# wei-zeng98/piano-a2s

Measured on AMD Instinct MI355X. Metric: training clips/sec (12 s, 5-bar), higher is better.
Workload: dtype f32

## Files before the change

piano_a2s_amd/csrc/a2s_api.hip:

```cpp
#define A2S_SWITCHES_IMPL
#include "a2s_internal.h"

thread_local char a2s_err_msg[512] = {0};
long long a2s_launch_counter = 0;

#define ST ((hipStream_t)stream)

extern "C" {

const char* a2s_last_error(void) { return a2s_err_msg; }
int a2s_version(void) { return 1; }
long long a2s_launch_count(void) { return __atomic_load_n(&a2s_launch_counter, __ATOMIC_RELAXED); }

int a2s_gemm_f32(void* stream, int M, int N, int K, float alpha, const float* A, long sAm, long sAk, const float* B, long sBk,
                 long sBn, float beta, float* C, long ldc, const float* bias, int act, int batch, long bsA, long bsB, long bsC,
                 int splitk, float* workspace, size_t workspace_bytes) {
    return a2s_gemm_impl(ST, M, N, K, alpha, A, sAm, sAk, B, sBk, sBn, beta, C, ldc, bias, act, batch, bsA, bsB, bsC, splitk,
                         workspace, workspace_bytes);
}
int a2s_gemm_f32_affine(void* stream, int M, int N, int K, float alpha, const float* A, long sAm, long sAk, const float* B, long sBk,
                        long sBn, float beta, float* C, long ldc, const float* bias, int act, int batch, long bsA, long bsB, long bsC,
                        int splitk, float* workspace, size_t workspace_bytes, const float* a_scale, const float* a_shift, int a_period,
                        const float* b_scale, const float* b_shift, int b_period) {
    return a2s_gemm_affine_impl(ST, M, N, K, alpha, A, sAm, sAk, B, sBk, sBn, beta, C, ldc, bias, act, batch, bsA, bsB, bsC, splitk,
                                workspace, workspace_bytes, a_scale, a_shift, a_period, b_scale, b_shift, b_period,
                                nullptr, nullptr, nullptr, nullptr, nullptr, nullptr, 0, 0, nullptr, nullptr);
}
int a2s_gemm_f32_affine_scaled(void* stream, int M, int N, int K, float alpha, const float* A, long sAm, long sAk, const float* B, long sBk,
                               long sBn, float beta, float* C, long ldc, const float* bias, int act, int batch, long bsA, long bsB, long bsC,
                               int splitk, float* workspace, size_t workspace_bytes, const float* a_scale, const float* a_shift, int a_period,
                               const float* b_scale, const float* b_shift, int b_period, const float* a_absmax, const float* b_absmax) {
    return a2s_gemm_affine_impl(ST, M, N, K, alpha, A, sAm, sAk, B, sBk, sBn, beta, C, ldc, bias, act, batch, bsA, bsB, bsC, splitk,
                                workspace, workspace_bytes, a_scale, a_shift, a_period, b_scale, b_shift, b_period,
                                nullptr, nullptr, nullptr, nullptr, nullptr, nullptr, 0, 1, a_absmax, b_absmax);
}
int a2s_gemm_f32_bnstats_scaled(void* stream, int M, int N, int K, const float* A, long sAm, long sAk, const float* B, long sBk, long sBn, float* C, long ldc,
                                const float* y, const float* mean, const float* invstd, const float* scale, const float* shift, int period, float* partial,
                                const float* a_absmax, const float* b_absmax) {
    return a2s_gemm_affine_impl(ST, M, N, K, 1.f, A, sAm, sAk, B, sBk, sBn, 0.f, C, ldc, nullptr, 0, 1, 0, 0, 0, 1, nullptr, 0,
                                nullptr, nullptr, 0, nullptr, nullptr, 0, y, mean, invstd, scale, shift, partial, period, 1, a_absmax, b_absmax);
}
int a2s_absmax(void* stream, const float* x, long n, float* out) { return a2s_absmax_impl(ST, x, n, out); }
int a2s_linear_dgrad_bnstats(void* stream, int M, int N, int K, const float* dz, long lda, const float* Wt, float* da, long ldc, const float* y,
                             const float* mean, const float* invstd, const float* scale, const float* shift, int period, float* partial,
                             const float* dz_absmax, const float* w_absmax, float* workspace, size_t workspace_bytes, float* da_absmax_out) {
    return a2s_linear_dgrad_bnstats_impl(ST, M, N, K, dz, lda, Wt, 1, K, da, ldc, y, mean, invstd, scale, shift, period, partial, dz_absmax, w_absmax,
                                         workspace, workspace_bytes, da_absmax_out);
}
size_t a2s_linear_dgrad_ws_bytes(int N, int K) { return a2s_linear_dgrad_ws_bytes_impl(N, K); }
int a2s_linear_fwd(void* stream, int M, int N, int K, const float* y, long lda, const float* W, float* z, long ldc, const float* scale, const float* shift,
                   int period, const float* y_absmax, const float* w_absmax, float* workspace, size_t workspace_bytes) {
    return a2s_linear_fwd_impl(ST, M, N, K, y, lda, W, z, ldc, scale, shift, period, y_absmax, w_absmax, workspace, workspace_bytes);
}
int a2s_linear_wgrad(void* stream, int M, int N, int K, const float* dz, long ldz, const float* y, long lda, float* G, long ldg, const float* scale,
                     const float* shift, int period, const float* dz_absmax, const float* y_absmax, float* workspace, size_t workspace_bytes) {
    return a2s_linear_wgrad_impl(ST, M, N, K, dz, ldz, y, lda, G, ldg, scale, shift, period, dz_absmax, y_absmax, workspace, workspace_bytes);
}
size_t a2s_linear_wgrad_ws_bytes(int M, int K) { return a2s_linear_wgrad_ws_bytes_impl(M, K); }
int a2s_linear_wgrad_eligible(int M, int N, int K, int period) { return a2s_linear_wgrad_ok(M, N, K, 256, 4, 4, period, nullptr, nullptr, nullptr) ? 1 : 0; }
int a2s_tallk_wgrad(void* stream, int M, int Np, int K, const float* P, long ldp, const float* A, long lda, float* G, long ldg, int transposed, float* bias,
                    const float* p_absmax, const float* a_absmax, float* workspace, size_t workspace_bytes) {
    return a2s_tallk_wgrad_impl(ST, M, Np, K, P, ldp, A, lda, G, ldg, transposed, bias, p_absmax, a_absmax, workspace, workspace_bytes);
}
size_t a2s_tallk_wgrad_ws_bytes(int M, int Np, int K) { return a2s_tallk_wgrad_ws_bytes_impl(M, Np, K); }
int a2s_tallk_wgrad_eligible(int M, int Np, int K, long ldp, long lda, long ldg, int transposed) {
    return a2s_tallk_wgrad_ok(M, Np, K, ldp, lda, ldg, transposed, nullptr, nullptr, nullptr, nullptr) ? 1 : 0;
}
int a2s_linear_fwd_eligible(int M, int N, int K, int period) { return a2s_linear_fwd_ok(M, N, K, 4, 4, period, nullptr, nullptr, nullptr) ? 1 : 0; }
int a2s_linear_dgrad_blocks(int M) { return a2s_linear_dgrad_blocks_impl(M); }
int a2s_linear_dgrad_eligible(int M, int N, int K, int period) {
    return a2s_linear_dgrad_ok(M, N, K, 4, 1, K, 4, period, nullptr, nullptr, nullptr, nullptr) ? 1 : 0;
}
int a2s_gemm_f32_bnstats(void* stream, int M, int N, int K, const float* A, long sAm, long sAk, const float* B, long sBk, long sBn, float* C, long ldc,
                         const float* y, const float* mean, const float* invstd, const float* scale, const float* shift, int period, float* partial) {
    return a2s_gemm_affine_impl(ST, M, N, K, 1.f, A, sAm, sAk, B, sBk, sBn, 0.f, C, ldc, nullptr, 0, 1, 0, 0, 0, 1, nullptr, 0,
                                nullptr, nullptr, 0, nullptr, nullptr, 0, y, mean, invstd, scale, shift, partial, period, 0, nullptr, nullptr);
}
int a2s_gemm_bnstats_blocks(int M, int period) { return a2s_cdiv(M, 128) * a2s_gemm_bnstats_slots(period); }
size_t a2s_gemm_workspace_bytes(int M, int N, int batch, int splitk) { return a2s_gemm_workspace_bytes_impl(M, N, batch, splitk); }
int a2s_gemm_pick_splitk(int M, int N, int K, int batch) { return a2s_gemm_pick_splitk_impl(M, N, K, batch); }
void a2s_gemm_debug_tile(int cfg) { a2s_gemm_debug_tile_impl(cfg); }
size_t a2s_note_step_workspace_floats(int H, int E) { return a2s_note_step_workspace_floats_impl(H, E); }
int a2s_debug_set(const char* key, int value) {
    if (!key) return A2S_ERR_ARG;
    const int id = a2s_switch_find(key);
    if (id >= 0) { a2s_switch_store(id, value); return A2S_OK; }
    if (!strcmp(key, "attn_deferred_fast")) { a2s_attn_deferred_fast = value ? 1 : 0; return A2S_OK; }
    if (!strcmp(key, "tallk_wgrad")) { a2s_tallk_wgrad_on = value ? 1 : 0; return A2S_OK; }
    if (!strcmp(key, "tallk_wgrad_max_splits")) { a2s_tallk_wgrad_max_splits = value > 0 ? value : 0; return A2S_OK; }
    if (!strcmp(key, "gemm_tile")) { a2s_gemm_debug_tile_impl(value); return A2S_OK; }
    snprintf(a2s_err_msg, sizeof(a2s_err_msg), "a2s_debug_set: unknown key %s", key);
    return A2S_ERR_ARG;
}
int a2s_env_check(void) {
    if (const char* e = a2s_switch_env_error()) A2S_FAIL(A2S_ERR_ARG, "%s: expected a decimal number >= 0", e);
    return A2S_OK;
}

int a2s_persist_abort_latch(void* device_word) { a2s_persist_latch_set(device_word); return A2S_OK; }

int a2s_debug_get(const char* key) {
    if (!key) return -1;
    const int id = a2s_switch_find(key);
    if (id == A2S_SW_attn_pair_fused_rows) return a2s_attn_pair_fused_rows();
    if (id >= 0) return a2s_sw((a2s_switch)id);
    if (!strcmp(key, "attn_pair_launches")) return (int)a2s_attn_pair_launches();
    if (!strcmp(key, "attn_pair_bwd_launches")) return (int)a2s_attn_pair_bwd_launches();
    if (!strcmp(key, "attn_deferred_fast")) return a2s_attn_deferred_fast;
    if (!strcmp(key, "tallk_wgrad")) return a2s_tallk_wgrad_on;
    if (!strcmp(key, "tallk_wgrad_max_splits")) return a2s_tallk_wgrad_max_splits;
    if (!strcmp(key, "tallk_wgrad_launches")) return (int)a2s_tallk_wgrad_launches();
    if (!strcmp(key, "attn_dk_ahead_launches")) return (int)a2s_attn_dk_ahead_launches();
    if (!strcmp(key, "attn_denc_launches")) return (int)a2s_attn_denc_launches();
    if (!strcmp(key, "dec_mid_launches")) return a2s_dec_mid_launches();
    if (!strcmp(key, "dec_persist_launches")) return a2s_dec_persist_launches();
    if (!strcmp(key, "edit_distance_launches")) return (int)a2s_edit_distance_launches();
    if (!strcmp(key, "conv_rows16_c20_launches")) return (int)a2s_conv_rows16_c20_launches();
    if (!strcmp(key, "device_cus")) return a2s_device_geometry().cus;
    if (!strcmp(key, "device_xccs")) return a2s_device_geometry().xccs;
    return -1;
}

int a2s_conv3x3(void* stream, const float* x, const float* w, float* y, const float* in_scale, const float* in_shift,
                float* stat_partial, int B, int T, int F, int Cin, int Cout, int flip, float* workspace) {
    return a2s_conv3x3_impl(ST, x, w, y, in_scale, in_shift, stat_partial, B, T, F, Cin, Cout, flip, workspace, nullptr, nullptr, nullptr, nullptr, nullptr, nullptr,
                            nullptr, nullptr);
}
int a2s_conv3x3_ranged(void* stream, const float* x, const float* w, float* y, const float* in_scale, const float* in_shift, const float* in_absmax,
                       float* stat_partial, float* out_absmax, int B, int T, int F, int Cin, int Cout, float* workspace) {
    return a2s_conv3x3_impl(ST, x, w, y, in_scale, in_shift, stat_partial, B, T, F, Cin, Cout, 0, workspace, nullptr, nullptr, nullptr, nullptr, nullptr, nullptr,
                            in_absmax, out_absmax);
}
int a2s_conv3x3_dgrad_bnstats(void* stream, const float* dy, const float* w, float* g, const float* yl, const float* yl_mean, const float* yl_invstd,
                              const float* yl_scale, const float* yl_shift, float* stat_partial, int B, int T, int F, int Cin, int Cout,
                              float* workspace) {
    if (!yl) { snprintf(a2s_err_msg, sizeof(a2s_err_msg), "conv3x3_dgrad_bnstats: yl is required"); return A2S_ERR_ARG; }
    return a2s_conv3x3_impl(ST, dy, w, g, nullptr, nullptr, stat_partial, B, T, F, Cin, Cout, 1, workspace, yl, yl_mean, yl_invstd, yl_scale, yl_shift, nullptr, nullptr, nullptr);
}
int a2s_conv3x3_dgrad_bnstats_scaled(void* stream, const float* dy, const float* w, float* g, const float* yl, const float* yl_mean, const float* yl_invstd,
                                     const float* yl_scale, const float* yl_shift, float* stat_partial, int B, int T, int F, int Cin, int Cout,
                                     float* workspace, const float* dy_absmax) {
    if (!yl) { snprintf(a2s_err_msg, sizeof(a2s_err_msg), "conv3x3_dgrad_bnstats_scaled: yl is required"); return A2S_ERR_ARG; }
    return a2s_conv3x3_impl(ST, dy, w, g, nullptr, nullptr, stat_partial, B, T, F, Cin, Cout, 1, workspace, yl, yl_mean, yl_invstd, yl_scale, yl_shift, dy_absmax, nullptr, nullptr);
}
int a2s_conv3x3_dgrad_bnstats_ranged(void* stream, const float* dy, const float* w, float* g, const float* yl, const float* yl_mean, const float* yl_invstd,
                                     const float* yl_scale, const float* yl_shift, float* stat_partial, int B, int T, int F, int Cin, int Cout,
                                     float* workspace, const float* dy_absmax, float* g_absmax_out) {
    if (!yl) { snprintf(a2s_err_msg, sizeof(a2s_err_msg), "conv3x3_dgrad_bnstats_ranged: yl is required"); return A2S_ERR_ARG; }
    return a2s_conv3x3_impl(ST, dy, w, g, nullptr, nullptr, stat_partial, B, T, F, Cin, Cout, 1, workspace, yl, yl_mean, yl_invstd, yl_scale, yl_shift, dy_absmax, nullptr, g_absmax_out);
}
int a2s_bn_bwd_from_partial(void* stream, const float* g, const float* x, const float* mean, const float* invstd, const float* scale, const float* shift,
                            float* dgamma, float* dbeta, float* dx, const float* partial, int nblocks, float* c12, long rows, int C, int F) {
    return a2s_bn_bwd_from_partial_impl(ST, g, x, mean, invstd, scale, shift, dgamma, dbeta, dx, partial, nblocks, c12, rows, C, F, nullptr);
}
int a2s_bn_bwd_from_partial_amax(void* stream, const float* g, const float* x, const float* mean, const float* invstd, const float* scale, const float* shift,
                                 float* dgamma, float* dbeta, float* dx, const float* partial, int nblocks, float* c12, long rows, int C, int F,
                                 float* dx_absmax) {
    return a2s_bn_bwd_from_partial_impl(ST, g, x, mean, invstd, scale, shift, dgamma, dbeta, dx, partial, nblocks, c12, rows, C, F, dx_absmax);
}
size_t a2s_conv3x3_workspace_floats(int Cin) { return a2s_conv3x3_workspace_floats_impl(Cin); }
int a2s_conv3x3_stat_blocks(int B, int T, int F, int Cin) { return a2s_conv3x3_stat_blocks_impl(B, T, F, Cin); }
int a2s_bn_finalize(void* stream, const float* partial, int nblocks, int C, double count, const float* gamma, const float* beta,
                    float* running_mean, float* running_var, long long* nbt, float* mean, float* invstd, float* scale,
                    float* shift, float eps, float momentum, int training) {
    return a2s_bn_finalize_impl(ST, partial, nblocks, C, count, gamma, beta, running_mean, running_var, nbt, mean, invstd, scale,
                                shift, eps, momentum, training);
}
int a2s_bn_relu_apply(void* stream, const float* x, float* y, const float* scale, const float* shift, long n, int C, int F) {
    return a2s_bn_relu_apply_impl(ST, x, y, scale, shift, n, C, F);
}
int a2s_col_stats(void* stream, const float* x, float* partial, long rows, int C, int rows_per_block) {
    return a2s_col_stats_impl(ST, x, partial, rows, C, rows_per_block);
}
int a2s_bn1d_relu_dropout(void* stream, const float* x, float* y, const float* scale, const float* shift, const uint8_t* keep_mask,
                          float inv_keep, long n, int C) {
    return a2s_bn1d_relu_dropout_impl(ST, x, y, scale, shift, keep_mask, inv_keep, n, C);
}
int a2s_gru_gates_fwd(void* stream, const float* gi, long ldgi, const float* gh, long ldgh, const float* hprev, long ldhp,
                      float* hout, long ldho, float* hout2, long ldho2, float* save, int R, int H) {
    return a2s_gru_gates_fwd_impl(ST, gi, ldgi, gh, ldgh, hprev, ldhp, hout, ldho, hout2, ldho2, save, R, H);
}
int a2s_gru_seq_fwd(void* stream, const float* gi_all, long gi_bstride, long gi_tstride, const float* w_hh, const float* b_hh,
                    float* out, long out_bstride, long out_tstride, float* hbuf, float* gh, float* save, float* hn, int B, int T,
                    int H, int reverse, float* workspace, size_t workspace_bytes) {
    return a2s_gru_seq_fwd_impl(ST, gi_all, gi_bstride, gi_tstride, w_hh, b_hh, out, out_bstride, out_tstride, hbuf, gh, save, hn,
                                B, T, H, reverse, workspace, workspace_bytes);
}
int a2s_attn_step_fwd(void* stream, const float* keys, const float* enc, const float* q, long ldq, const float* v, float* ctx,
                      long ldctx, float* ctx2, long ldctx2, float* attw, int B, int T, int H, const int* n_done, int n_rows_total, float* workspace) {
    return a2s_attn_step_fwd_impl(ST, keys, enc, q, ldq, v, ctx, ldctx, ctx2, ldctx2, attw, B, T, H, n_done, n_rows_total, workspace, nullptr);
}
int a2s_attn_step_fwd_rows(void* stream, const float* keys, const float* enc, const float* q, long ldq, const float* v, float* ctx,
                           long ldctx, float* ctx2, long ldctx2, float* attw, int R, int T, int H, float* workspace, int n_clips,
                           const int* clip_order, const int* clip_rank, const int* row_until, int n_active, int step) {
// ... 258 lines not shown
```

piano_a2s_amd/csrc/a2s_internal.h:

```cpp
#pragma once
#include "a2s_common.h"
#include "../../include/a2s.h"
#include "a2s_switches.h"

static inline int a2s_attn_pair_fused_rows(void) {
    const int cap = a2s_sw(A2S_SW_dec_fused_max_rows), v = a2s_sw(A2S_SW_attn_pair_fused_rows);
    return v < cap ? v : cap;
}
static inline unsigned a2s_persist_dbg(void) {
    return (a2s_sw(A2S_SW_persist_force_agent) ? PERSIST_DBG_FORCE_AGENT : 0u) | (a2s_sw(A2S_SW_persist_inject_abort) ? PERSIST_DBG_INJECT_ABORT : 0u);
}

int a2s_absmax_impl(hipStream_t st, const float* x, long n, float* out);
size_t a2s_gemm_workspace_bytes_impl(int M, int N, int batch, int splitk);
int a2s_gemm_pick_splitk_impl(int M, int N, int K, int batch);
int a2s_gemm_bnstats_slots(int period);
void a2s_gemm_debug_tile_impl(int cfg);
int a2s_gemm_affine_impl(hipStream_t st, int M, int N, int K, float alpha, const float* A, long sAm, long sAk,
    const float* B, long sBk, long sBn, float beta, float* C, long ldc, const float* bias, int act,
    int batch, long bsA, long bsB, long bsC, int splitk, float* ws, size_t ws_bytes,
    const float* a_scale, const float* a_shift, int a_period, const float* b_scale, const float* b_shift, int b_period,
    const float* ep_y, const float* ep_mean, const float* ep_invstd, const float* ep_scale, const float* ep_shift,
    float* ep_partial, int ep_period, int two_term, const float* a_absmax, const float* b_absmax);
int a2s_gemm_impl(hipStream_t st, int M, int N, int K, float alpha, const float* A, long sAm, long sAk,
    const float* B, long sBk, long sBn, float beta, float* C, long ldc, const float* bias, int act,
    int batch, long bsA, long bsB, long bsC, int splitk, float* ws, size_t ws_bytes);

size_t a2s_linear_dgrad_ws_bytes_impl(int N, int K);
int a2s_linear_dgrad_blocks_impl(int M);
bool a2s_linear_dgrad_ok(int M, int N, int K, long lda, long sBk, long sBn, long ldc, int period, const void* A, const void* B, const void* C, const void* y);
int a2s_linear_dgrad_bnstats_impl(hipStream_t st, int M, int N, int K, const float* A, long lda, const float* Wt, long sBk, long sBn, float* C, long ldc,
    const float* ep_y, const float* mean, const float* invstd, const float* scale, const float* shift, int period,
    float* partial, const float* a_absmax, const float* b_absmax, float* ws, size_t ws_bytes, float* c_absmax_out);
bool a2s_linear_fwd_ok(int M, int N, int K, long lda, long ldc, int period, const void* A, const void* W, const void* C);
int a2s_linear_fwd_impl(hipStream_t st, int M, int N, int K, const float* A, long lda, const float* W, float* C, long ldc, const float* a_scale,
    const float* a_shift, int period, const float* a_absmax, const float* w_absmax, float* ws, size_t ws_bytes);
size_t a2s_linear_wgrad_ws_bytes_impl(int M, int K);
bool a2s_linear_wgrad_ok(int M, int N, int K, long ldz, long lda, long ldg, int period, const void* dz, const void* A, const void* G);
int a2s_linear_wgrad_impl(hipStream_t st, int M, int N, int K, const float* dz, long ldz, const float* A, long lda, float* G, long ldg, const float* a_scale,
    const float* a_shift, int period, const float* dz_absmax, const float* a_absmax, float* ws, size_t ws_bytes);
extern int a2s_tallk_wgrad_on;
extern int a2s_tallk_wgrad_max_splits;
long a2s_tallk_wgrad_launches(void);
size_t a2s_tallk_wgrad_ws_bytes_impl(int M, int Np, int K);
bool a2s_tallk_wgrad_ok(int M, int Np, int K, long ldp, long lda, long ldg, int transposed, const void* P, const void* A, const void* G, const void* bias);
int a2s_tallk_wgrad_impl(hipStream_t st, int M, int Np, int K, const float* P, long ldp, const float* A, long lda, float* G, long ldg, int transposed,
    float* bias, const float* p_absmax, const float* a_absmax, float* ws, size_t ws_bytes);

int a2s_act_bound_impl(hipStream_t st, const float* scale, const float* shift, const float* absmax, int C, float* out);
size_t a2s_conv3x3_workspace_floats_impl(int Cin);
int a2s_conv3x3_impl(hipStream_t st, const float* x, const float* w, float* y, const float* in_scale,
    const float* in_shift, float* stat_partial, int B, int T, int F, int Cin, int Cout, int flip, float* ws,
    const float* yl, const float* yl_mean, const float* yl_invstd, const float* yl_scale, const float* yl_shift,
    const float* x_absmax, const float* in_absmax, float* out_absmax);
int a2s_conv3x3_stat_blocks_impl(int B, int T, int F, int Cin);
int a2s_bn_finalize_impl(hipStream_t st, const float* partial, int nblocks, int C, double count, const float* gamma,
    const float* beta, float* running_mean, float* running_var, long long* nbt, float* mean,
    float* invstd, float* scale, float* shift, float eps, float momentum, int training);
int a2s_bn_relu_apply_impl(hipStream_t st, const float* x, float* y, const float* scale, const float* shift, long n, int C, int F);
int a2s_col_stats_impl(hipStream_t st, const float* x, float* partial, long rows, int C, int rows_per_block);
int a2s_bn1d_relu_dropout_impl(hipStream_t st, const float* x, float* y, const float* scale, const float* shift,
    const uint8_t* mask, float inv_keep, long n, int C);
size_t a2s_conv3x3_wgrad_workspace_bytes_impl(int Cin, int Cout);
int a2s_conv3x3_wgrad_impl(hipStream_t st, const float* dy, const float* x, const float* in_scale, const float* in_shift, float* dW,
    float* ws, size_t ws_bytes, int B, int T, int F, int Cin, int Cout, const float* bn_y, const float* bn_mean,
    const float* bn_invstd, const float* bn_scale, const float* bn_shift, const float* bn_c12, float* dy_out,
    const float* dy_absmax, const float* act_absmax);
int a2s_bn_bwd_impl(hipStream_t st, const float* g, const float* x, const float* mean, const float* invstd, const float* scale,
    const float* shift, const uint8_t* mask, float inv_keep, float* dgamma, float* dbeta, float* dx, float* partial,
    float* c12, long rows, int C, int F, float* dx_absmax);
int a2s_bn_bwd_from_partial_impl(hipStream_t st, const float* g, const float* x, const float* mean, const float* invstd, const float* scale,
    const float* shift, float* dgamma, float* dbeta, float* dx, const float* partial, int nblocks, float* c12,
    long rows, int C, int F, float* dx_absmax);
int a2s_bn_bwd_stats_impl(hipStream_t st, const float* g, const float* x, const float* mean, const float* invstd, const float* scale,
    const float* shift, const uint8_t* mask, float inv_keep, float* partial, float* sums, long rows, int C, int F);
int a2s_bn_bwd_apply_impl(hipStream_t st, const float* g, const float* x, const float* mean, const float* invstd, const float* scale,
    const float* shift, const uint8_t* mask, float inv_keep, const float* sums_local, const float* sums_global,
    double count_global, float* dgamma, float* dbeta, float* dx, float* c12, long rows, int C, int F);
int a2s_bn_bwd_sums_from_partial_impl(hipStream_t st, const float* partial, int nblocks, int C, float* sums);
int a2s_bn_bwd_c12_from_sums_impl(hipStream_t st, const float* sums_local, const float* sums_global, double count_global, float* dgamma, float* dbeta,
    float* c12, int C);
size_t a2s_bn_bwd_partial_floats_impl(long rows, int C, int F);

int a2s_channel_absmax_impl(hipStream_t st, const float* x, long rows, int C, int F, float* out);
bool a2s_conv_rows_eligible(int F, int Cin);
int a2s_conv_rows_blocks(int B, int T, int F);
size_t a2s_conv_rows_workspace_floats(int Cin);
long a2s_conv_rows16_c20_launches(void);
int a2s_conv3x3_rows_impl(hipStream_t st, const float* x, const float* w, float* y, const float* in_scale, const float* in_shift,
    const float* in_absmax, float* stat_partial, float* out_absmax, int B, int T, int F, int Cin, int Cout, int flip,
    float* ws, const float* yl, const float* yl_mean, const float* yl_invstd, const float* yl_scale, const float* yl_shift,
    const float* x_absmax);

bool a2s_wgrad_rows_eligible(int F, int Cin, int Cout);
int a2s_conv3x3_wgrad_rows_bn_impl(hipStream_t st, const float* g, const float* y, const float* mean, const float* invstd, const float* scale,
    const float* shift, const float* c12, const float* g_absmax, int g_absmax_n, const float* y_absmax, float* dz_out,
    float* dz_absmax_out, const float* x, const float* in_scale, const float* in_shift, float* dW, float* ws, size_t ws_bytes,
    int B, int T, int F, int Cin, int Cout, const float* act_absmax);
int a2s_conv3x3_wgrad_rows_impl(hipStream_t st, const float* dy, const float* x, const float* in_scale, const float* in_shift, float* dW, float* ws,
    size_t ws_bytes, int B, int T, int F, int Cin, int Cout, const float* dy_absmax, const float* act_absmax);

struct StepFinArgs {
    const float* logits; long ldl;
    float* probs; long probs_bstride;
    const long long* gt; long gt_bstride;
    const float* emb;
    float* xnext; long ldx;
    const uint8_t* drop; float inv_keep;
    int* argmax_out; long am_bstride;
    int* eos_seen; long long* lengths; int* n_done; int* steps_exec;
    const int* t_base;
    const int* row_until;
    int n_clips;
    int R, V, E, t, teacher_force, eos_id, max_t;
};
struct a2s_grammar_ref { const signed char* next; int n_states; int* row_state; };
int a2s_gru_gates_fwd_impl(hipStream_t st, const float* gi, long ldgi, const float* gh, long ldgh, const float* hprev,
    long ldhp, float* hout, long ldho, float* hout2, long ldho2, float* save, int R, int H);
int a2s_gru_bptt_step_impl(hipStream_t st, const float* dgh, const float* w_hh_t, const float* dhz_in, const float* dout, long ld_dout,
    const float* save, const float* hprev, long ld_hprev, float* dgi, long ld_dgi, float* dgh_out, float* dgh2,
    long ld_dgh2, float* dhz_out, int R, int H);
int a2s_skinny_gemm_acc_impl(hipStream_t st, const float* A, long lda, const float* Bt, long ldb, float* Cm, long ldc, int R, int N, int K);
int a2s_gru_seq_fwd_impl(hipStream_t st, const float* gi_all, long gi_bstride, long gi_tstride, const float* w_hh,
    const float* b_hh, float* out, long out_bstride, long out_tstride, float* hbuf, float* gh,
    float* save, float* hn, int B, int T, int H, int reverse, float* ws, size_t ws_bytes);
int a2s_attn_step_fwd_impl(hipStream_t st, const float* Kmat, const float* enc, const float* q, long ldq, const float* v,
// ... 161 lines not shown
```

piano_a2s_amd/csrc/a2s_linear.hip:

```cpp
#include "a2s_internal.h"

#define LIN_BM 128
#define LIN_K 256
#define LIN_RS 288
#define LIN_NTH 512
#define LIN_LDS (2 * 2 * LIN_BM * LIN_RS)

typedef unsigned lu32x4 __attribute__((ext_vector_type(4)));

struct LinDgradArgs {
    const float* A; long lda;
    const unsigned char* planes;
    float* C; long ldc;
    const float* ep_y;
    const float* mean; const float* invstd; const float* scale; const float* shift;
    float* partial;
    const float* a_absmax; const float* b_absmax;
    int M, N, period, channels;
    float* c_absmax_out;
};

__global__ __launch_bounds__(256) void lin_pack_planes_k(const float* __restrict__ W, long ld, int N, int K, const float* __restrict__ absmax,
                                                         unsigned char* __restrict__ out) {
    const long id = (long)blockIdx.x * 256 + threadIdx.x;
// ... 264 lines not shown
#pragma unroll
        for (int sp = 0; sp < 2; ++sp)
#pragma unroll
            for (int q = 0; q < 2; ++q) af[sp][q] = *reinterpret_cast<const lu32x4*>(st + (sp * LIN_BM + (qt * 2 + q) * 16 + lr) * LF_RS + h * 64 + lk * 16);
    };
    auto multiply = [&](int qt, const lu32x4 (&af)[2][2], const lu32x4 (&b)[4][2]) {
#define LR_PRODUCT(SA, SB)                                                                                                        \
        _Pragma("unroll") for (int nt = 0; nt < 4; ++nt)                                                                          \
            _Pragma("unroll") for (int q = 0; q < 2; ++q)                                                                         \
                acc[qt * 2 + q][nt] = __builtin_amdgcn_mfma_f32_16x16x32_f16(__builtin_bit_cast(f16x8, b[nt][SB]),                \
                                                                             __builtin_bit_cast(f16x8, af[SA][q]), acc[qt * 2 + q][nt], 0, 0, 0);
        LR_PRODUCT(1, 0) LR_PRODUCT(0, 1) LR_PRODUCT(0, 0)
#undef LR_PRODUCT
    };
#pragma unroll 1
    for (int blk = 0; blk < nblk; ++blk) {
        __syncthreads();
        const unsigned char* st = lds + (blk % LF_NS) * LF_STAGE;
        lu32x4 fa[2][2], fb[2][2];
        load_af(st, 0, 0, fa);
        load_b(2 * blk + 1, bf[1]);
        __builtin_amdgcn_sched_barrier(0);
        load_af(st, 0, 1, fb); multiply(0, fa, bf[0]);
        __builtin_amdgcn_sched_barrier(0);
        load_af(st, 0, 2, fa); multiply(1, fb, bf[0]);
        __builtin_amdgcn_sched_barrier(0);
        load_af(st, 0, 3, fb); multiply(2, fa, bf[0]);
        __builtin_amdgcn_sched_barrier(0);
        load_af(st, 1, 0, fa); multiply(3, fb, bf[0]);
        __builtin_amdgcn_sched_barrier(0);
        load_b(2 * blk + 2, bf[0]);
        load_af(st, 1, 1, fb); multiply(0, fa, bf[1]);
        __builtin_amdgcn_sched_barrier(0);
        load_af(st, 1, 2, fa); multiply(1, fb, bf[1]);
        __builtin_amdgcn_sched_barrier(0);
        load_af(st, 1, 3, fb); multiply(2, fa, bf[1]);
        __builtin_amdgcn_sched_barrier(0);
        multiply(3, fb, bf[1]);
        __builtin_amdgcn_sched_barrier(0);
    }
#pragma unroll
    for (int mt = 0; mt < 8; ++mt) {
        const int m = m0 + mt * 16 + lr;
        if (m >= a.M) continue;
#pragma unroll
        for (int nt = 0; nt < 4; ++nt) {
            f32x4 v = acc[mt][nt];
#pragma unroll
            for (int r = 0; r < 4; ++r) v[r] *= unscale;
            *reinterpret_cast<f32x4*>(a.C + (long)m * a.ldc + wave * 64 + nt * 16 + lk * 4) = v;
        }
    }
}

bool a2s_linear_fwd_ok(int M, int N, int K, long lda, long ldc, int period, const void* A, const void* W, const void* C) {
    return N == 256 && M >= 1 && K >= 128 && K % 64 == 0 && (period == 0 || (period % 32 == 0 && K % period == 0)) && lda % 4 == 0 && ldc % 4 == 0 &&
           (((uintptr_t)A | (uintptr_t)W | (uintptr_t)C) % 16 == 0);
}

int a2s_linear_fwd_impl(hipStream_t st, int M, int N, int K, const float* A, long lda, const float* W, float* C, long ldc, const float* a_scale,
                        const float* a_shift, int period, const float* a_absmax, const float* w_absmax, float* ws, size_t ws_bytes) {
    A2S_REQUIRE(A && W && C && w_absmax && ws && ((a_scale == nullptr) == (a_shift == nullptr)), "linear_fwd: null argument");
    A2S_REQUIRE(a2s_linear_fwd_ok(M, N, K, lda, ldc, a_scale ? period : 0, A, W, C),
                "linear_fwd: needs N = 256, K %% 64 == 0, period %% 32 == 0 and 16-byte aligned rows");
    A2S_REQUIRE(((uintptr_t)ws % 16 == 0) && ws_bytes >= (size_t)N * K * 4, "linear_fwd: workspace too small (%zu bytes needed)", (size_t)N * K * 4);
    unsigned char* planes = reinterpret_cast<unsigned char*>(ws);
    hipLaunchKernelGGL(lin_pack_planes_k, dim3((unsigned)(((long)N * (K / 8) + 255) / 256)), dim3(256), 0, st, W, (long)K, N, K, w_absmax, planes);
    A2S_CHECK_LAUNCH("lin_pack_planes_k");
    LinFwdArgs a{A, lda, planes, C, ldc, a_scale, a_shift, a_absmax, w_absmax, M, K, a_scale ? period : K};
    hipLaunchKernelGGL(lin_fwd_roles, dim3((M + LIN_BM - 1) / LIN_BM), dim3(LIN_NTH), 0, st, a);
    A2S_CHECK_LAUNCH("lin_fwd");
    return A2S_OK;
}

struct LinWgradArgs {
    const float* A; long lda;
    const unsigned char* planes;
    float* partial;
    const float* a_scale; const float* a_shift;
    const float* a_absmax; const float* d_absmax;
    int M, K, period, nblk, blk_per_split;
    long plane_stride; int np;
    float* bias_partial;
};

__global__ __launch_bounds__(256) void lin_pack_dz_planes(const float* __restrict__ dz, long ld, int M, int nsteps, const float* __restrict__ absmax,
                                                          unsigned char* __restrict__ out) {
    const long id = (long)blockIdx.x * 256 + threadIdx.x;
    const int n = (int)(id & 255), lk = (int)((id >> 8) & 3), s = (int)(id >> 10);
    if (s >= nsteps) return;
    dz += blockIdx.y * 256;
    out += (size_t)blockIdx.y * nsteps * (16 * 2 * 1024);
    float ps = ldexpf(1.f, pow2_scale_exp(*absmax, 12));
    if ((s >> 3) & 1) ps = -ps;
    float x[8];
#pragma unroll
    for (int j = 0; j < 8; ++j) {
        const int m = s * 32 + lk * 8 + j;
        x[j] = m < M ? __builtin_amdgcn_fmed3f(dz[(long)m * ld + n] * ps, -65000.f, 65000.f) : 0.f;
    }
    lu32x4 hi, lo;
#pragma unroll
    for (int i = 0; i < 4; ++i) { unsigned h, l; split2_pair_f16(x[2 * i], x[2 * i + 1], h, l); hi[i] = h; lo[i] = l; }
    unsigned char* o = out + ((((long)s * 16 + (n >> 4)) * 2) * 64 + (lk * 16 + (n & 15))) * 16;
    *reinterpret_cast<lu32x4*>(o) = hi;
    *reinterpret_cast<lu32x4*>(o + 64 * 16) = lo;
}

template <bool BIAS>
__global__ __launch_bounds__(LIN_NTH) void lin_wgrad_roles(LinWgradArgs a) {
    __shared__ __attribute__((aligned(16))) unsigned char lds[LF_NS * LF_STAGE];
    const int tid = threadIdx.x, lane = tid & 63, lr = lane & 15, lk = lane >> 4;
    const int wave = __builtin_amdgcn_readfirstlane(tid >> 6);
    const int k0 = blockIdx.x * LIN_BM;
    const int b_lo = blockIdx.y * a.blk_per_split, b_hi = min(a.nblk, b_lo + a.blk_per_split);
    const int ka = a.a_absmax ? pow2_scale_exp(*a.a_absmax, 12) : 0, kd = pow2_scale_exp(*a.d_absmax, 12);
    const float psa = ldexpf(1.f, ka), unscale = ldexpf(1.f, -(ka + kd));
    const bool affine = a.a_scale != nullptr;
    if (wave >= 4) {
        const int st_ = tid - 256;
        const int rq = st_ & 15, cq0 = st_ >> 4;
        float sc[2], sh[2];
#pragma unroll
        for (int u = 0; u < 2; ++u) {
            const int ch = affine ? (k0 + 4 * (cq0 + 16 * u)) / a.period : 0;
            sc[u] = affine ? a.a_scale[ch] * psa : psa; sh[u] = affine ? a.a_shift[ch] * psa : 0.f;
        }
        const float floor_ = affine ? 0.f : -INFINITY;
        f32x4 ar[2][8];
        f32x4 bs[2] = {(f32x4){0.f, 0.f, 0.f, 0.f}, (f32x4){0.f, 0.f, 0.f, 0.f}};
        auto issue_a = [&](int blk, f32x4 (&r)[8]) {
#pragma unroll
            for (int u = 0; u < 2; ++u)
#pragma unroll
                for (int j = 0; j < 4; ++j) {
                    const int m = blk * 64 + 4 * rq + j;
                    r[4 * u + j] = (f32x4){0.f, 0.f, 0.f, 0.f};
                    if (m < a.M && blk < b_hi) r[4 * u + j] = __builtin_nontemporal_load(reinterpret_cast<const f32x4*>(a.A + (long)m * a.lda + k0 + 4 * (cq0 + 16 * u)));
                }
        };
        auto commit_a = [&](int blk, const f32x4 (&r)[8]) {
            if (blk >= b_hi) return;
            unsigned char* st = lds + (blk % LF_NS) * LF_STAGE;
            if (BIAS) {
#pragma unroll
                for (int u = 0; u < 2; ++u)
#pragma unroll
                    for (int j = 0; j < 4; ++j)
#pragma unroll
                        for (int c = 0; c < 4; ++c) bs[u][c] += r[4 * u + j][c];
            }
#pragma unroll
            for (int u = 0; u < 2; ++u)
#pragma unroll
                for (int c = 0; c < 4; ++c) {
                    float x[4];
#pragma unroll
                    for (int j = 0; j < 4; ++j) x[j] = __builtin_amdgcn_fmed3f(fmaxf(fmaf(r[4 * u + j][c], sc[u], sh[u]), floor_), -65000.f, 65000.f);
                    uint2 hi, lo;
                    split2_pair_f16(x[0], x[1], hi.x, lo.x);
                    split2_pair_f16(x[2], x[3], hi.y, lo.y);
                    *reinterpret_cast<uint2*>(st + (0 * LIN_BM + 4 * (cq0 + 16 * u) + c) * LF_RS + rq * 8) = hi;
                    *reinterpret_cast<uint2*>(st + (1 * LIN_BM + 4 * (cq0 + 16 * u) + c) * LF_RS + rq * 8) = lo;
                }
        };
        if (b_lo < b_hi) {
            issue_a(b_lo, ar[0]);
            commit_a(b_lo, ar[0]);
            issue_a(b_lo + 1, ar[1]); issue_a(b_lo + 2, ar[0]);
        }
#pragma unroll 1
        for (int b = b_lo; b < b_hi; b += 2) {
            __syncthreads();
            commit_a(b + 1, ar[1]); issue_a(b + 3, ar[1]);
            if (b + 1 < b_hi) {
                __syncthreads();
                commit_a(b + 2, ar[0]); issue_a(b + 4, ar[0]);
            }
        }
        if (BIAS && blockIdx.z == 0) {
#pragma unroll
            for (int u = 0; u < 2; ++u) {
#pragma unroll
                for (int c = 0; c < 4; ++c)
#pragma unroll
                    for (int o = 1; o < 16; o <<= 1) bs[u][c] += __shfl_xor(bs[u][c], o, 64);
                if (rq == 0) *reinterpret_cast<f32x4*>(a.bias_partial + (long)blockIdx.y * a.K + k0 + 4 * (cq0 + 16 * u)) = bs[u];
            }
        }
        return;
    }
    lu32x4 df[2][4][2];
    const unsigned char* planes = a.planes + blockIdx.z * a.plane_stride;
    auto load_d = [&](int step, lu32x4 (&dst)[4][2]) {
        if (step >= 2 * b_hi) return;
#pragma unroll
        for (int nt = 0; nt < 4; ++nt)
#pragma unroll
            for (int sp = 0; sp < 2; ++sp)
                dst[nt][sp] = *reinterpret_cast<const lu32x4*>(planes + ((((long)step) * 16 + wave * 4 + nt) * 2 + sp) * 1024 + (unsigned)lane * 16u);
    };
    f32x4 acc[8][4];
#pragma unroll
    for (int kt = 0; kt < 8; ++kt)
#pragma unroll
        for (int nt = 0; nt < 4; ++nt) acc[kt][nt] = (f32x4){0.f, 0.f, 0.f, 0.f};
    bool neg = false;
    auto flip = [&]() {
#pragma unroll
        for (int kt = 0; kt < 8; ++kt)
#pragma unroll
            for (int nt = 0; nt < 4; ++nt)
#pragma unroll
                for (int r = 0; r < 4; ++r) acc[kt][nt][r] = -acc[kt][nt][r];
    };
    auto load_bf = [&](const unsigned char* st, int h, int qt, lu32x4 (&f)[2][2]) {
#pragma unroll
        for (int sp = 0; sp < 2; ++sp)
#pragma unroll
            for (int q = 0; q < 2; ++q) f[sp][q] = *reinterpret_cast<const lu32x4*>(st + (sp * LIN_BM + (qt * 2 + q) * 16 + lr) * LF_RS + h * 64 + lk * 16);
    };
    auto multiply = [&](int qt, const lu32x4 (&f)[2][2], const lu32x4 (&d)[4][2]) {
#define LW_PRODUCT(SX, SD)                                                                                                        \
        _Pragma("unroll") for (int nt = 0; nt < 4; ++nt)                                                                          \
            _Pragma("unroll") for (int q = 0; q < 2; ++q)                                                                         \
                acc[qt * 2 + q][nt] = __builtin_amdgcn_mfma_f32_16x16x32_f16(__builtin_bit_cast(f16x8, f[SX][q]),                 \
                                                                             __builtin_bit_cast(f16x8, d[nt][SD]), acc[qt * 2 + q][nt], 0, 0, 0);
        LW_PRODUCT(1, 0) LW_PRODUCT(0, 1) LW_PRODUCT(0, 0)
#undef LW_PRODUCT
    };
    load_d(2 * b_lo, df[0]);
#pragma unroll 1
    for (int blk = b_lo; blk < b_hi; ++blk) {
        const bool want = ((2 * blk) >> 3) & 1;
        if (want != neg) { flip(); neg = want; }
        __syncthreads();
        const unsigned char* st = lds + (blk % LF_NS) * LF_STAGE;
        lu32x4 fa[2][2], fb[2][2];
        load_bf(st, 0, 0, fa);
        load_d(2 * blk + 1, df[1]);
        __builtin_amdgcn_sched_barrier(0);
        load_bf(st, 0, 1, fb); multiply(0, fa, df[0]);
        __builtin_amdgcn_sched_barrier(0);
        load_bf(st, 0, 2, fa); multiply(1, fb, df[0]);
        __builtin_amdgcn_sched_barrier(0);
        load_bf(st, 0, 3, fb); multiply(2, fa, df[0]);
        __builtin_amdgcn_sched_barrier(0);
        load_bf(st, 1, 0, fa); multiply(3, fb, df[0]);
        __builtin_amdgcn_sched_barrier(0);
        load_d(2 * blk + 2, df[0]);
        load_bf(st, 1, 1, fb); multiply(0, fa, df[1]);
        __builtin_amdgcn_sched_barrier(0);
        load_bf(st, 1, 2, fa); multiply(1, fb, df[1]);
        __builtin_amdgcn_sched_barrier(0);
        load_bf(st, 1, 3, fb); multiply(2, fa, df[1]);
        __builtin_amdgcn_sched_barrier(0);
        multiply(3, fb, df[1]);
        __builtin_amdgcn_sched_barrier(0);
    }
    if (neg) flip();
    float* slab = a.partial + ((long)blockIdx.y * a.np + blockIdx.z * 256) * a.K;
#pragma unroll
    for (int kt = 0; kt < 8; ++kt)
#pragma unroll
        for (int nt = 0; nt < 4; ++nt) {
            f32x4 v = acc[kt][nt];
#pragma unroll
            for (int r = 0; r < 4; ++r) v[r] *= unscale;
            *reinterpret_cast<f32x4*>(slab + (long)(wave * 64 + nt * 16 + lr) * a.K + k0 + kt * 16 + lk * 4) = v;
        }
}

template <bool TR>
__global__ __launch_bounds__(256) void lin_wgrad_reduce(const float* __restrict__ partial, int splits, long n, float* __restrict__ G, long ldg, int K,
                                                        const float* __restrict__ bias_partial, float* __restrict__ bias) {
    const long i = ((long)blockIdx.x * 256 + threadIdx.x) * 4;
    if (i >= n) {
        const long k = i - n;
        if (!bias_partial || k >= K) return;
        f32x4 s = *reinterpret_cast<const f32x4*>(bias_partial + k);
        for (int p = 1; p < splits; ++p) {
            const f32x4 v = *reinterpret_cast<const f32x4*>(bias_partial + (long)p * K + k);
#pragma unroll
            for (int r = 0; r < 4; ++r) s[r] += v[r];
        }
#pragma unroll
        for (int r = 0; r < 4; ++r) bias[k + r] += s[r];
        return;
    }
    f32x4 s = *reinterpret_cast<const f32x4*>(partial + i);
    for (int p = 1; p < splits; ++p) {
        const f32x4 v = *reinterpret_cast<const f32x4*>(partial + (long)p * n + i);
#pragma unroll
        for (int r = 0; r < 4; ++r) s[r] += v[r];
    }
    if (TR) {
        float* g = G + (i % K) * ldg + (i / K);
#pragma unroll
        for (int r = 0; r < 4; ++r) g[r * ldg] += s[r];
        return;
    }
    float* g = G + (i / K) * ldg + (i % K);
    const f32x4 o = *reinterpret_cast<const f32x4*>(g);
#pragma unroll
    for (int r = 0; r < 4; ++r) s[r] += o[r];
    *reinterpret_cast<f32x4*>(g) = s;
}

static int lin_wgrad_splits(int M, int K) {
    const int ncol = K / LIN_BM, nblk = (M + 63) / 64;
    int s = (768 + ncol - 1) / ncol;
    if (s > 16) s = 16;
    if (s > nblk) s = nblk;
    return s < 1 ? 1 : s;
}
size_t a2s_linear_wgrad_ws_bytes_impl(int M, int K) {
    if (M < 1 || K < LIN_BM || K % LIN_BM) return 0;
    const size_t nsteps = 2 * (size_t)((M + 63) / 64);
    return nsteps * 16 * 2 * 1024 + (size_t)lin_wgrad_splits(M, K) * 256 * K * sizeof(float);
}
bool a2s_linear_wgrad_ok(int M, int N, int K, long ldz, long lda, long ldg, int period, const void* dz, const void* A, const void* G) {
    return N == 256 && M >= 64 && K >= LIN_BM && K % LIN_BM == 0 && (period == 0 || (period % 4 == 0 && K % period == 0)) && lda % 4 == 0 && ldg % 4 == 0 && ldz >= 256 &&
           (((uintptr_t)dz | (uintptr_t)A | (uintptr_t)G) % 16 == 0);
}
int a2s_linear_wgrad_impl(hipStream_t st, int M, int N, int K, const float* dz, long ldz, const float* A, long lda, float* G, long ldg, const float* a_scale,
                          const float* a_shift, int period, const float* dz_absmax, const float* a_absmax, float* ws, size_t ws_bytes) {
    A2S_REQUIRE(dz && A && G && dz_absmax && ws && ((a_scale == nullptr) == (a_shift == nullptr)), "linear_wgrad: null argument");
    A2S_REQUIRE(a2s_linear_wgrad_ok(M, N, K, ldz, lda, ldg, a_scale ? period : 0, dz, A, G), "linear_wgrad: needs N = 256, K %% 128 == 0, period %% 4 == 0, 16-byte aligned rows");
    A2S_REQUIRE(((uintptr_t)ws % 16 == 0) && ws_bytes >= a2s_linear_wgrad_ws_bytes_impl(M, K), "linear_wgrad: workspace too small (%zu bytes needed)",
                a2s_linear_wgrad_ws_bytes_impl(M, K));
    const int nblk = (M + 63) / 64, nsteps = 2 * nblk, splits = lin_wgrad_splits(M, K);
    unsigned char* planes = reinterpret_cast<unsigned char*>(ws);
    float* partial = reinterpret_cast<float*>(planes + (size_t)nsteps * 16 * 2 * 1024);
    hipLaunchKernelGGL(lin_pack_dz_planes, dim3((unsigned)(((long)nsteps * 1024 + 255) / 256)), dim3(256), 0, st, dz, ldz, M, nsteps, dz_absmax, planes);
    A2S_CHECK_LAUNCH("lin_pack_dz_planes");
    LinWgradArgs a{A, lda, planes, partial, a_scale, a_shift, a_absmax, dz_absmax, M, K, a_scale ? period : K, nblk, (nblk + splits - 1) / splits, 0, 256, nullptr};
    hipLaunchKernelGGL(lin_wgrad_roles<false>, dim3(K / LIN_BM, splits), dim3(LIN_NTH), 0, st, a);
    A2S_CHECK_LAUNCH("lin_wgrad");
    const long n = 256L * K;
    hipLaunchKernelGGL(lin_wgrad_reduce<false>, dim3((unsigned)((n / 4 + 255) / 256)), dim3(256), 0, st, partial, splits, n, G, ldg, K, nullptr, nullptr);
    A2S_CHECK_LAUNCH("lin_wgrad_reduce");
    return A2S_OK;
}

#define TALLK_SLAB_BYTES (64u << 20)
int a2s_tallk_wgrad_on = 1;
int a2s_tallk_wgrad_max_splits = 0;
static long long g_tallk_launches = 0;
long a2s_tallk_wgrad_launches(void) { return (long)__atomic_load_n(&g_tallk_launches, __ATOMIC_RELAXED); }

static int tallk_splits(int M, int Np, int K) {
    const int tiles = (K / LIN_BM) * (Np / 256), nblk = (M + 63) / 64;
    int cus = a2s_device_geometry().cus;
    if (cus < 1) cus = 256;
    int s = cus / tiles;
    const size_t slab = (size_t)Np * K * sizeof(float);
    if ((size_t)s * slab > TALLK_SLAB_BYTES) s = (int)(TALLK_SLAB_BYTES / slab);
    if (s > nblk) s = nblk;
    if (a2s_tallk_wgrad_max_splits > 0 && s > a2s_tallk_wgrad_max_splits) s = a2s_tallk_wgrad_max_splits;
    return s < 1 ? 1 : s;
}
bool a2s_tallk_wgrad_ok(int M, int Np, int K, long ldp, long lda, long ldg, int transposed, const void* P, const void* A, const void* G, const void* bias) {
    return a2s_tallk_wgrad_on && M >= 64 && Np >= 256 && Np % 256 == 0 && Np <= 2048 && K >= LIN_BM && K % LIN_BM == 0 && K <= 4096 && ldp >= Np && lda >= K &&
           lda % 4 == 0 && ldg % 4 == 0 && ldg >= (transposed ? Np : K) && (((uintptr_t)P | (uintptr_t)A | (uintptr_t)G | (uintptr_t)bias) % 16 == 0);
}
size_t a2s_tallk_wgrad_ws_bytes_impl(int M, int Np, int K) {
    if (M < 1 || Np < 256 || Np % 256 || K < LIN_BM || K % LIN_BM) return 0;
    const size_t nsteps = 2 * (size_t)((M + 63) / 64), splits = (size_t)tallk_splits(M, Np, K);
    return (size_t)(Np / 256) * nsteps * 16 * 2 * 1024 + splits * Np * K * sizeof(float) + splits * K * sizeof(float);
}
int a2s_tallk_wgrad_impl(hipStream_t st, int M, int Np, int K, const float* P, long ldp, const float* A, long lda, float* G, long ldg, int transposed,
                         float* bias, const float* p_absmax, const float* a_absmax, float* ws, size_t ws_bytes) {
    A2S_REQUIRE(P && A && G && p_absmax && a_absmax && ws, "tallk_wgrad: null argument");
    A2S_REQUIRE(a2s_tallk_wgrad_ok(M, Np, K, ldp, lda, ldg, transposed, P, A, G, bias),
                "tallk_wgrad: needs M >= 64, Np %% 256 == 0, K %% 128 == 0, 16-byte aligned bases and rows (or the switch \"tallk_wgrad\" is off)");
    A2S_REQUIRE(((uintptr_t)ws % 16 == 0) && ws_bytes >= a2s_tallk_wgrad_ws_bytes_impl(M, Np, K), "tallk_wgrad: workspace too small (%zu bytes needed)",
                a2s_tallk_wgrad_ws_bytes_impl(M, Np, K));
    const int nblk = (M + 63) / 64, nsteps = 2 * nblk, splits = tallk_splits(M, Np, K), npb = Np / 256;
    const size_t plane_stride = (size_t)nsteps * 16 * 2 * 1024;
    unsigned char* planes = reinterpret_cast<unsigned char*>(ws);
    float* partial = reinterpret_cast<float*>(planes + npb * plane_stride);
    float* bias_partial = partial + (size_t)splits * Np * K;
    hipLaunchKernelGGL(lin_pack_dz_planes, dim3((unsigned)(((long)nsteps * 1024 + 255) / 256), npb), dim3(256), 0, st, P, ldp, M, nsteps, p_absmax, planes);
    A2S_CHECK_LAUNCH("lin_pack_dz_planes");
    LinWgradArgs a{A, lda, planes, partial, nullptr, nullptr, a_absmax, p_absmax, M, K, K, nblk, (nblk + splits - 1) / splits, (long)plane_stride, Np,
                   bias ? bias_partial : nullptr};
    if (bias) hipLaunchKernelGGL(lin_wgrad_roles<true>, dim3(K / LIN_BM, splits, npb), dim3(LIN_NTH), 0, st, a);
    else hipLaunchKernelGGL(lin_wgrad_roles<false>, dim3(K / LIN_BM, splits, npb), dim3(LIN_NTH), 0, st, a);
    A2S_CHECK_LAUNCH("lin_wgrad (tall-K)");
    const long n = (long)Np * K, nthreads = (n + (bias ? K : 0)) / 4;
    const dim3 rgrid((unsigned)((nthreads + 255) / 256));
    if (transposed) hipLaunchKernelGGL(lin_wgrad_reduce<true>, rgrid, dim3(256), 0, st, partial, splits, n, G, ldg, K, bias ? bias_partial : nullptr, bias);
    else hipLaunchKernelGGL(lin_wgrad_reduce<false>, rgrid, dim3(256), 0, st, partial, splits, n, G, ldg, K, bias ? bias_partial : nullptr, bias);
    A2S_CHECK_LAUNCH("lin_wgrad_reduce");
    __atomic_fetch_add(&g_tallk_launches, 1LL, __ATOMIC_RELAXED);
    return A2S_OK;
}
```

Measured before the change: 641.3.

## Make linear weight-grad kernel persistent with range-major work-item scheduling

Turns the lin_wgrad_roles kernel into a persistent kernel. A grid sized to the number of resident workgroups loops over flattened (column, split-range, plane) work items, ordered range-major, instead of launching one workgroup per tile. The aim is to cut tail-wave imbalance and improve locality of the shared dz planes across items. An optional, default-off 'even' mode picks split counts that fill whole rounds of resident workgroups. The cost is an extra barrier between items, and prefetching the A tile before that barrier adds some ordering risk.

```diff
diff --git a/piano_a2s_amd/csrc/a2s_api.hip b/piano_a2s_amd/csrc/a2s_api.hip
--- a/piano_a2s_amd/csrc/a2s_api.hip
+++ b/piano_a2s_amd/csrc/a2s_api.hip
@@ -88,6 +88,9 @@
     if (!strcmp(key, "attn_deferred_fast")) { a2s_attn_deferred_fast = value ? 1 : 0; return A2S_OK; }
     if (!strcmp(key, "tallk_wgrad")) { a2s_tallk_wgrad_on = value ? 1 : 0; return A2S_OK; }
     if (!strcmp(key, "tallk_wgrad_max_splits")) { a2s_tallk_wgrad_max_splits = value > 0 ? value : 0; return A2S_OK; }
+    if (!strcmp(key, "lin_wgrad_sched")) { a2s_lin_wgrad_sched = value ? 1 : 0; return A2S_OK; }
+    if (!strcmp(key, "lin_wgrad_even")) { a2s_lin_wgrad_even = value > 0 ? value : 0; return A2S_OK; }
+    if (!strcmp(key, "lin_wgrad_sched_max_wgs")) { a2s_lin_wgrad_sched_max_wgs = value > 0 ? value : 0; return A2S_OK; }
     if (!strcmp(key, "gemm_tile")) { a2s_gemm_debug_tile_impl(value); return A2S_OK; }
     snprintf(a2s_err_msg, sizeof(a2s_err_msg), "a2s_debug_set: unknown key %s", key);
     return A2S_ERR_ARG;
@@ -110,6 +113,10 @@
     if (!strcmp(key, "tallk_wgrad")) return a2s_tallk_wgrad_on;
     if (!strcmp(key, "tallk_wgrad_max_splits")) return a2s_tallk_wgrad_max_splits;
     if (!strcmp(key, "tallk_wgrad_launches")) return (int)a2s_tallk_wgrad_launches();
+    if (!strcmp(key, "lin_wgrad_sched")) return a2s_lin_wgrad_sched;
+    if (!strcmp(key, "lin_wgrad_even")) return a2s_lin_wgrad_even;
+    if (!strcmp(key, "lin_wgrad_sched_max_wgs")) return a2s_lin_wgrad_sched_max_wgs;
+    if (!strcmp(key, "lin_wgrad_sched_launches")) return (int)a2s_lin_wgrad_sched_launches();
     if (!strcmp(key, "attn_dk_ahead_launches")) return (int)a2s_attn_dk_ahead_launches();
     if (!strcmp(key, "attn_denc_launches")) return (int)a2s_attn_denc_launches();
     if (!strcmp(key, "dec_mid_launches")) return a2s_dec_mid_launches();
diff --git a/piano_a2s_amd/csrc/a2s_internal.h b/piano_a2s_amd/csrc/a2s_internal.h
--- a/piano_a2s_amd/csrc/a2s_internal.h
+++ b/piano_a2s_amd/csrc/a2s_internal.h
@@ -42,6 +42,10 @@
 extern int a2s_tallk_wgrad_on;
 extern int a2s_tallk_wgrad_max_splits;
 long a2s_tallk_wgrad_launches(void);
+extern int a2s_lin_wgrad_sched;
+extern int a2s_lin_wgrad_even;
+extern int a2s_lin_wgrad_sched_max_wgs;
+long a2s_lin_wgrad_sched_launches(void);
 size_t a2s_tallk_wgrad_ws_bytes_impl(int M, int Np, int K);
 bool a2s_tallk_wgrad_ok(int M, int Np, int K, long ldp, long lda, long ldg, int transposed, const void* P, const void* A, const void* G, const void* bias);
 int a2s_tallk_wgrad_impl(hipStream_t st, int M, int Np, int K, const float* P, long ldp, const float* A, long lda, float* G, long ldg, int transposed,
diff --git a/piano_a2s_amd/csrc/a2s_linear.hip b/piano_a2s_amd/csrc/a2s_linear.hip
--- a/piano_a2s_amd/csrc/a2s_linear.hip
+++ b/piano_a2s_amd/csrc/a2s_linear.hip
@@ -370,6 +370,8 @@
     int M, K, period, nblk, blk_per_split;
     long plane_stride; int np;
     float* bias_partial;
+    int ncol, splits, npb, nitems;
+    int range_major;
 };
 
 __global__ __launch_bounds__(256) void lin_pack_dz_planes(const float* __restrict__ dz, long ld, int M, int nsteps, const float* __restrict__ absmax,
@@ -400,12 +402,19 @@
     __shared__ __attribute__((aligned(16))) unsigned char lds[LF_NS * LF_STAGE];
     const int tid = threadIdx.x, lane = tid & 63, lr = lane & 15, lk = lane >> 4;
     const int wave = __builtin_amdgcn_readfirstlane(tid >> 6);
-    const int k0 = blockIdx.x * LIN_BM;
-    const int b_lo = blockIdx.y * a.blk_per_split, b_hi = min(a.nblk, b_lo + a.blk_per_split);
     const int ka = a.a_absmax ? pow2_scale_exp(*a.a_absmax, 12) : 0, kd = pow2_scale_exp(*a.d_absmax, 12);
     const float psa = ldexpf(1.f, ka), unscale = ldexpf(1.f, -(ka + kd));
     const bool affine = a.a_scale != nullptr;
+    const int first = (int)(blockIdx.x + gridDim.x * (blockIdx.y + gridDim.y * blockIdx.z)), nwg = (int)(gridDim.x * gridDim.y * gridDim.z);
+#define LW_ITEM_DECODE                                                                                                                    \
+    const int col = item % a.ncol, rest = item / a.ncol;                                                                                  \
+    const int range = a.range_major ? rest / a.npb : rest % a.splits, pblk = a.range_major ? rest % a.npb : rest / a.splits;              \
+    const int k0 = col * LIN_BM;                                                                                                          \
+    const int b_lo = range * a.blk_per_split, b_hi = min(a.nblk, b_lo + a.blk_per_split);
     if (wave >= 4) {
+#pragma unroll 1
+      for (int item = first; item < a.nitems; item += nwg) {
+        LW_ITEM_DECODE
         const int st_ = tid - 256;
         const int rq = st_ & 15, cq0 = st_ >> 4;
         float sc[2], sh[2];
@@ -452,8 +461,9 @@
                     *reinterpret_cast<uint2*>(st + (1 * LIN_BM + 4 * (cq0 + 16 * u) + c) * LF_RS + rq * 8) = lo;
                 }
         };
+        issue_a(b_lo, ar[0]);
+        if (item != first) __syncthreads();
         if (b_lo < b_hi) {
-            issue_a(b_lo, ar[0]);
             commit_a(b_lo, ar[0]);
             issue_a(b_lo + 1, ar[1]); issue_a(b_lo + 2, ar[0]);
         }
@@ -466,20 +476,24 @@
                 commit_a(b + 2, ar[0]); issue_a(b + 4, ar[0]);
             }
         }
-        if (BIAS && blockIdx.z == 0) {
+        if (BIAS && pblk == 0) {
 #pragma unroll
             for (int u = 0; u < 2; ++u) {
 #pragma unroll
                 for (int c = 0; c < 4; ++c)
 #pragma unroll
                     for (int o = 1; o < 16; o <<= 1) bs[u][c] += __shfl_xor(bs[u][c], o, 64);
-                if (rq == 0) *reinterpret_cast<f32x4*>(a.bias_partial + (long)blockIdx.y * a.K + k0 + 4 * (cq0 + 16 * u)) = bs[u];
-            }
-        }
-        return;
-    }
+                if (rq == 0) *reinterpret_cast<f32x4*>(a.bias_partial + (long)range * a.K + k0 + 4 * (cq0 + 16 * u)) = bs[u];
+            }
+        }
+      }
+      return;
+    }
+#pragma unroll 1
+    for (int item = first; item < a.nitems; item += nwg) {
+    LW_ITEM_DECODE
     lu32x4 df[2][4][2];
-    const unsigned char* planes = a.planes + blockIdx.z * a.plane_stride;
+    const unsigned char* planes = a.planes + pblk * a.plane_stride;
     auto load_d = [&](int step, lu32x4 (&dst)[4][2]) {
         if (step >= 2 * b_hi) return;
 #pragma unroll
@@ -518,6 +532,7 @@
 #undef LW_PRODUCT
     };
     load_d(2 * b_lo, df[0]);
+    if (item != first) __syncthreads();
 #pragma unroll 1
     for (int blk = b_lo; blk < b_hi; ++blk) {
         const bool want = ((2 * blk) >> 3) & 1;
@@ -547,7 +562,7 @@
         __builtin_amdgcn_sched_barrier(0);
     }
     if (neg) flip();
-    float* slab = a.partial + ((long)blockIdx.y * a.np + blockIdx.z * 256) * a.K;
+    float* slab = a.partial + ((long)range * a.np + pblk * 256) * a.K;
 #pragma unroll
     for (int kt = 0; kt < 8; ++kt)
 #pragma unroll
@@ -557,6 +572,8 @@
             for (int r = 0; r < 4; ++r) v[r] *= unscale;
             *reinterpret_cast<f32x4*>(slab + (long)(wave * 64 + nt * 16 + lr) * a.K + k0 + kt * 16 + lk * 4) = v;
         }
+    }
+#undef LW_ITEM_DECODE
 }
 
 template <bool TR>
@@ -595,12 +612,59 @@
     *reinterpret_cast<f32x4*>(g) = s;
 }
 
+#define LIN_WGRAD_EVEN_MAX_SPLITS 17
+#define TALLK_EVEN_MIN_BLOCKS 16
+int a2s_lin_wgrad_sched = 1;
+int a2s_lin_wgrad_even = 0;
+int a2s_lin_wgrad_sched_max_wgs = 0;
+static long long g_lin_wgrad_sched_launches = 0;
+long a2s_lin_wgrad_sched_launches(void) { return (long)__atomic_load_n(&g_lin_wgrad_sched_launches, __ATOMIC_RELAXED); }
+
+static int lin_wgrad_resident(void) {
+    static int per_cu = -1;
+    if (per_cu < 0) {
+        int n = 0;
+        if (hipOccupancyMaxActiveBlocksPerMultiprocessor(&n, lin_wgrad_roles<true>, LIN_NTH, 0) != hipSuccess) { (void)hipGetLastError(); n = 0; }
+        per_cu = n < 1 ? 1 : n;
+    }
+    int cus = a2s_device_geometry().cus;
+    if (cus < 1) cus = 256;
+    return cus * per_cu;
+}
+template <bool BIAS>
+static void lin_wgrad_launch(hipStream_t st, LinWgradArgs a) {
+    a.nitems = a.ncol * a.splits * a.npb;
+    if (!a2s_lin_wgrad_sched) {
+        a.range_major = 0;
+        hipLaunchKernelGGL(lin_wgrad_roles<BIAS>, dim3(a.ncol, a.splits, a.npb), dim3(LIN_NTH), 0, st, a);
+        return;
+    }
+    a.range_major = 1;
+    int wgs = lin_wgrad_resident();
+    if (a2s_lin_wgrad_sched_max_wgs > 0 && wgs > a2s_lin_wgrad_sched_max_wgs) wgs = a2s_lin_wgrad_sched_max_wgs;
+    if (wgs > a.nitems) wgs = a.nitems;
+    hipLaunchKernelGGL(lin_wgrad_roles<BIAS>, dim3(wgs), dim3(LIN_NTH), 0, st, a);
+    __atomic_fetch_add(&g_lin_wgrad_sched_launches, 1LL, __ATOMIC_RELAXED);
+}
+
 static int lin_wgrad_splits(int M, int K) {
     const int ncol = K / LIN_BM, nblk = (M + 63) / 64;
     int s = (768 + ncol - 1) / ncol;
     if (s > 16) s = 16;
     if (s > nblk) s = nblk;
-    return s < 1 ? 1 : s;
+    if (s < 1) s = 1;
+    const int wgs = lin_wgrad_resident();
+    if (a2s_lin_wgrad_even > 0 && ncol * s > wgs) {
+        int best = s;
+        double best_fill = 0.0;
+        for (int c = s; c <= LIN_WGRAD_EVEN_MAX_SPLITS && c <= nblk; ++c) {
+            const int items = ncol * c, rounds = (items + wgs - 1) / wgs;
+            const double fill = (double)items / ((double)rounds * wgs);
+            if (fill > best_fill + 1e-9) { best_fill = fill; best = c; }
+        }
+        s = best;
+    }
+    return s;
 }
 size_t a2s_linear_wgrad_ws_bytes_impl(int M, int K) {
     if (M < 1 || K < LIN_BM || K % LIN_BM) return 0;
@@ -622,8 +686,9 @@
     float* partial = reinterpret_cast<float*>(planes + (size_t)nsteps * 16 * 2 * 1024);
     hipLaunchKernelGGL(lin_pack_dz_planes, dim3((unsigned)(((long)nsteps * 1024 + 255) / 256)), dim3(256), 0, st, dz, ldz, M, nsteps, dz_absmax, planes);
     A2S_CHECK_LAUNCH("lin_pack_dz_planes");
-    LinWgradArgs a{A, lda, planes, partial, a_scale, a_shift, a_absmax, dz_absmax, M, K, a_scale ? period : K, nblk, (nblk + splits - 1) / splits, 0, 256, nullptr};
-    hipLaunchKernelGGL(lin_wgrad_roles<false>, dim3(K / LIN_BM, splits), dim3(LIN_NTH), 0, st, a);
+    LinWgradArgs a{A, lda, planes, partial, a_scale, a_shift, a_absmax, dz_absmax, M, K, a_scale ? period : K, nblk, (nblk + splits - 1) / splits, 0, 256, nullptr,
+                   K / LIN_BM, splits, 1, 0, 0};
+    lin_wgrad_launch<false>(st, a);
     A2S_CHECK_LAUNCH("lin_wgrad");
     const long n = 256L * K;
     hipLaunchKernelGGL(lin_wgrad_reduce<false>, dim3((unsigned)((n / 4 + 255) / 256)), dim3(256), 0, st, partial, splits, n, G, ldg, K, nullptr, nullptr);
@@ -642,6 +707,10 @@
     int cus = a2s_device_geometry().cus;
     if (cus < 1) cus = 256;
     int s = cus / tiles;
+    if (a2s_lin_wgrad_even > 0) {
+        const int more = (int)((long)a2s_lin_wgrad_even * lin_wgrad_resident() / tiles), longest = nblk / TALLK_EVEN_MIN_BLOCKS;
+        if (more > s) s = more < longest ? more : (longest > s ? longest : s);
+    }
     const size_t slab = (size_t)Np * K * sizeof(float);
     if ((size_t)s * slab > TALLK_SLAB_BYTES) s = (int)(TALLK_SLAB_BYTES / slab);
     if (s > nblk) s = nblk;
@@ -672,9 +741,9 @@
     hipLaunchKernelGGL(lin_pack_dz_planes, dim3((unsigned)(((long)nsteps * 1024 + 255) / 256), npb), dim3(256), 0, st, P, ldp, M, nsteps, p_absmax, planes);
     A2S_CHECK_LAUNCH("lin_pack_dz_planes");
     LinWgradArgs a{A, lda, planes, partial, nullptr, nullptr, a_absmax, p_absmax, M, K, K, nblk, (nblk + splits - 1) / splits, (long)plane_stride, Np,
-                   bias ? bias_partial : nullptr};
-    if (bias) hipLaunchKernelGGL(lin_wgrad_roles<true>, dim3(K / LIN_BM, splits, npb), dim3(LIN_NTH), 0, st, a);
-    else hipLaunchKernelGGL(lin_wgrad_roles<false>, dim3(K / LIN_BM, splits, npb), dim3(LIN_NTH), 0, st, a);
+                   bias ? bias_partial : nullptr, K / LIN_BM, splits, npb, 0, 0};
+    if (bias) lin_wgrad_launch<true>(st, a);
+    else lin_wgrad_launch<false>(st, a);
     A2S_CHECK_LAUNCH("lin_wgrad (tall-K)");
     const long n = (long)Np * K, nthreads = (n + (bias ? K : 0)) / 4;
     const dim3 rgrid((unsigned)((nthreads + 255) / 256));
```

New measurement: 640.3. Within noise of the previous version (-0.2%).
